# Zhang-Xiaoxue/Senquential-Convex-Programming-for-Trajectory-Planning

Measured on AMD Instinct MI355X. Metric: SCP-QP solves/sec/GPU (4 veh, Hp=20); traj ℓ∞ err vs CVXOPT, higher is better.
Workload: dtype f64; 1 GPU; c2: 4-vehicle circle/crossing, Hp=20, batch=1024 noise seeds per GPU, full SCP solve per problem; n_veh=4, hp=20, batch_per_gpu=1024, parallelism=1 independent shards (no collective)

## Files before the change

senquential-convex-programming-for-trajectory-planning_amd/csrc/scpqp_kernel.h:

```cpp

#pragma once

#include <hip/hip_runtime.h>

#include <math.h>
#include <stdint.h>
#include <stdio.h>
#include <stdlib.h>
#include <string.h>

#include <new>
#include <type_traits>
#include <utility>

#include "scpqp.h"

#define NT 256
#define TXD 16
#define TYD (NT / TXD)
#define NWAVE (NT / 64)
#define SCR_PER_WAVE 640

namespace {

// ... 1208 lines not shown
            if (u2 == 1 && tb == t) break;
            const int i0 = r1 + 2 * ia[u2], k0 = r1 + 2 * ka[u2];
            const int o0 = roff(i0), o1 = roff(i0 + 1);
            const double f = NEUTRAL ? 0.0 : 1.0;
            H[o0 + k0] -= f * sm[u2][0];
            H[o0 + k0 + 1] -= f * sm[u2][1];
            H[o1 + k0] -= f * sm[u2][2];
            H[o1 + k0 + 1] -= f * sm[u2][3];
        }
    }
}

typedef double double4v __attribute__((ext_vector_type(4)));

template <int U, int KS, class HP>
__device__ __forceinline__ void trailing_update_mfma(HP H, int n, int j0, int r1, const ldouble* dcur,
                                                     int wave, int nwave, int part = 0, int np = 1) {
    const int lane = threadIdx.x & 63, lr = lane & 15, lk = lane >> 4;
    double dk[KS];
#pragma unroll
    for (int kk = 0; kk < KS; ++kk) dk[kk] = dcur[4 * kk + lk];
    const int T = (n - r1 + 15) >> 4;
    const int ntile = T * (T + 1) / 2;
    int tb = 0, te = ntile;
    if (part != 0) {
        int js = 1, cum = T;
        for (int k = 1; k < np; ++k) {
            while (js < T && np * cum < k * ntile) {
                cum += T - js;
                ++js;
            }
            if (k == part - 1) tb = cum;
            if (k == part) te = cum;
        }
    }
    for (int t = tb + wave; t < te; t += U * nwave) {
        double a[U][KS], b[U][KS];
        double4v acc[U];
        int oc[U][4];
        bool ok[U][4];
#pragma unroll
        for (int u = 0; u < U; ++u) {
            const int tu = t + u * nwave;
            const bool live = tu < te;
            int I = 0, J = 0;
            tri_decode(ntile - 1 - (live ? tu : t), J, I);
            I = T - 1 - I;
            J = T - 1 - J;
            const int i0 = r1 + 16 * I, k0 = r1 + 16 * J;
            const int ia = min(i0 + lr, n - 1), kb = min(k0 + lr, n - 1);
            const int oa = roff(ia) + j0, ob = roff(kb) + j0;
#pragma unroll
            for (int kk = 0; kk < KS; ++kk) {
                a[u][kk] = -H[oa + 4 * kk + lk] * dk[kk];
                b[u][kk] = H[ob + 4 * kk + lk];
            }
            const int kc = k0 + lr;
#pragma unroll
            for (int r = 0; r < 4; ++r) {
                const int ci = i0 + lk + 4 * r;
                ok[u][r] = live && ci < n && kc <= ci;
                oc[u][r] = roff(ok[u][r] ? ci : 0) + (ok[u][r] ? kc : 0);
                acc[u][r] = ok[u][r] ? (double)H[oc[u][r]] : 0.0;
            }
        }
#pragma unroll
        for (int u = 0; u < U; ++u) {
#pragma unroll
            for (int kk = 0; kk < KS; ++kk)
                acc[u] = __builtin_amdgcn_mfma_f64_16x16x4f64(a[u][kk], b[u][kk], acc[u], 0, 0, 0);
        }
#pragma unroll
        for (int u = 0; u < U; ++u)
#pragma unroll
            for (int r = 0; r < 4; ++r)
                if (ok[u][r]) H[oc[u][r]] = acc[u][r];
    }
}

constexpr int kGroup = 4;
static_assert(kPivSlot + 2 * kGroup * CB == red_size(true) && kPivSlot + 2 * CB == red_size(false),
              "the pivot buffer of red_size");

template <class LT>
__device__ bool cholesky(const LT& L) {
    const int n = __builtin_amdgcn_readfirstlane(L.n);
    constexpr int RS = LT::RMAX;
    constexpr int G = LT::HGLOBAL ? kGroup : 1;
    lint* flag = (lint*)(L.red + kRedFlag);
    ldouble* ldbuf = L.red;
    ldouble* dbuf = L.red + kPivSlot;
    PROF_T0();
    for (int r0 = 0, s = 0; r0 < n; r0 += CB, ++s) {
        const int par = s & 1;
        const int jb = min(CB, n - r0), r1 = r0 + jb;
        const int sg = s % G;
        const int np = G == 1 ? 1 : (sg == 0 ? G : sg);
        const int jp = r0 - np * CB;
        const ldouble* dprev = dbuf + ((s - np) & (2 * G - 1)) * CB;
        if (is_lead(L.lead)) {
            ldouble* dn = dbuf + (s % (2 * G)) * CB;
            lead_prio_up();
            constexpr bool OPQ = RS > 2;
            if (RS == 1 || n - r0 <= 64) panel_factor<1, OPQ>(L.H, L.dinv, n, r0, jb, jp, dprev, dn, flag + par, np, ldbuf);
            else panel_factor<RS, OPQ>(L.H, L.dinv, n, r0, jb, jp, dprev, dn, flag + par, np, ldbuf);
            lead_prio_down();
        } else if (jp >= 0 || (G > 1 && s >= G)) {
            const int tw = (wave_id() - L.lead + NWAVE - 1) % NWAVE;
            if constexpr (LT::HGLOBAL) {
                constexpr int U = 2;
                const int s0 = s - sg;
                if (s0 >= G)
                    trailing_update_mfma<U, G * CB / 4>(L.H, n, (s0 - G) * CB, s0 * CB + CB,
                                                        dbuf + ((s0 - G) & (2 * G - 1)) * CB,
                                                        tw, NWAVE - 1, sg + 1, G);
            } else {
                trailing_update(L.H, n, jp, r1, dprev, tw * 64 + (int)(threadIdx.x & 63), NT - 64);
#ifdef SCPQP_DIAG_X2_TRAIL
                trailing_update<decltype(L.H), true>(L.H, n, jp, r1, dprev, tw * 64 + (int)(threadIdx.x & 63), NT - 64);
#endif
            }
        }
#if defined(SCPQP_PROF) && defined(SCPQP_PROF_FINE)
        unsigned long long _pb = __builtin_amdgcn_s_memtime();
#endif
        bar();
#if defined(SCPQP_PROF) && defined(SCPQP_PROF_FINE)
        if (threadIdx.x == 64 * L.lead) atomicAdd(&g_prof[22], __builtin_amdgcn_s_memtime() - _pb);
        if (threadIdx.x == 64 * ((L.lead + 1) & 3)) atomicAdd(&g_prof[23], __builtin_amdgcn_s_memtime() - _pb);
#endif
        if (flag[par]) return false;
    }
    PROF_ACC(13);
    return true;
}


constexpr int kSolveChunk = 4;
constexpr int kSolveChunkG = 8;
template <int LN, int LP>
__device__ __forceinline__ double bcast_capture_d(double v, double& dst, int& blo, int& bhi) {
    static_assert(LN >= 0 && LN < 64 && LP < 64, "lanes of the wave");
    const long long b = __double_as_longlong(v);
    const int vlo = static_cast<int>(b & 0xffffffffll), vhi = static_cast<int>(b >> 32);
    int lo, hi;
    if constexpr (LP >= 0) {
        const long long d = __double_as_longlong(dst);
        int dlo = static_cast<int>(d & 0xffffffffll), dhi = static_cast<int>(d >> 32);
        asm("s_nop 0\n\tv_readlane_b32 %0, %4, %8\n\tv_readlane_b32 %1, %5, %8\n\t"
            "v_writelane_b32 %2, %6, %9\n\tv_writelane_b32 %3, %7, %9"
            : "=&s"(lo), "=&s"(hi), "+v"(dlo), "+v"(dhi)
            : "v"(vlo), "v"(vhi), "s"(blo), "s"(bhi), "i"(LN), "i"(LP));
        dst = __longlong_as_double((static_cast<long long>(dhi) << 32) | static_cast<unsigned int>(dlo));
    } else {
        asm("s_nop 0\n\tv_readlane_b32 %0, %2, %4\n\tv_readlane_b32 %1, %3, %4\n\ts_nop 1"
            : "=&s"(lo), "=&s"(hi)
            : "v"(vlo), "v"(vhi), "i"(LN));
    }
    blo = lo;
    bhi = hi;
    return __longlong_as_double((static_cast<long long>(hi) << 32) | static_cast<unsigned int>(lo));
}
template <int LP>
__device__ __forceinline__ void flush_lane_d(double& dst, int blo, int bhi) {
    static_assert(LP >= 0 && LP < 64, "a lane of the wave");
    const long long d = __double_as_longlong(dst);
    int dlo = static_cast<int>(d & 0xffffffffll), dhi = static_cast<int>(d >> 32);
    asm("v_writelane_b32 %0, %2, %4\n\tv_writelane_b32 %1, %3, %4"
        : "+v"(dlo), "+v"(dhi)
        : "s"(blo), "s"(bhi), "i"(LP));
    dst = __longlong_as_double((static_cast<long long>(dhi) << 32) | static_cast<unsigned int>(dlo));
}
template <int R, class HP, int SCH, int NC = 0>
struct Solver {
    static constexpr bool RTN = NC == 0;
    static_assert(SCH % 2 == 0 && 64 % SCH == 0, "chunks tile the 64-row slots");
    static_assert(NC <= 64 * R, "every row has a slot");
    HP H;
    const ldouble* dinv;
    int lane, n, ld;
    double r[R], xf[R];
    int ii[R], ro[R], ic[R];
    double cur[R][SCH], nxt[R][SCH];

    __device__ __forceinline__ Solver(HP H_, const ldouble* dinv_, int n_, int ld_,
                                      const ldouble* bvec)
        : H(H_), dinv(dinv_), n(n_), ld(ld_) {
        lane = threadIdx.x & 63;
#pragma unroll
        for (int t = 0; t < R; ++t) {
            ii[t] = lane + 64 * t;
            ic[t] = ii[t] < n ? ii[t] : n - 1;
            ro[t] = roff(ic[t]);
            r[t] = ii[t] < n ? bvec[ii[t]] : 0.0;
            xf[t] = 0.0;
        }
    }
    __device__ __forceinline__ void load_cols(double (&dst)[R][SCH], int jc) {
#pragma unroll
        for (int t = 0; t < R; ++t)
#pragma unroll
            for (int q = 0; q < SCH; q += 2) {
                const double2v v = ld2(H + ro[t] + jc + q);
                dst[t][q] = v.x;
                dst[t][q + 1] = v.y;
            }
    }
    __device__ __forceinline__ void load_rows(double (&dst)[R][SCH], int jc) {
#pragma unroll
        for (int q = 0; q < SCH; ++q) {
            const int row = jc + q < n ? jc + q : n - 1;
#pragma unroll
            for (int t = 0; t < R; ++t) dst[t][q] = H[roff(row) + ic[t]];
        }
    }
// ... 25 lines not shown
    template <int T, int... C>
    __device__ __forceinline__ void fwd_chunks(std::integer_sequence<int, C...>) {
        (fwd_chunk<T, 64 * T + SCH * C>(std::make_integer_sequence<int, SCH>{}), ...);
    }
    template <int T, int J, int Q>
    __device__ __forceinline__ void bwd_step() {
        if constexpr (J < NC) {
            constexpr int jfirst = NC - 1 < 64 * T + 63 ? NC - 1 : 64 * T + 63;
            const double xj = bcast_capture_d<(J & 63), (J == jfirst ? -1 : ((J + 1) & 63))>(r[T], xf[T], blo, bhi);
            r[T] -= cur[T][Q] * xj;
#pragma unroll
            for (int t = 0; t < T; ++t) r[t] -= cur[t][Q] * xj;
        }
    }
    template <int T, int JC, int... Q>
    __device__ __forceinline__ void bwd_chunk(std::integer_sequence<int, Q...>) {
        if constexpr (JC > 0) load_rows(nxt, JC - SCH);
        (bwd_step<T, JC + SCH - 1 - Q, SCH - 1 - Q>(), ...);
        shift();
    }
    template <int T, int JSTART, int... C>
    __device__ __forceinline__ void bwd_chunks(std::integer_sequence<int, C...>) {
        (bwd_chunk<T, JSTART - SCH * C>(std::make_integer_sequence<int, SCH>{}), ...);
    }
    template <int T>
    __device__ __forceinline__ void fwd() {
        if constexpr (T < R && !RTN) {
            constexpr int jend = NC < 64 * (T + 1) ? NC : 64 * (T + 1);
            constexpr int nch = jend > 64 * T ? (jend - 64 * T + SCH - 1) / SCH : 0;
            fwd_chunks<T>(std::make_integer_sequence<int, nch>{});
            if constexpr (nch > 0) flush_lane_d<((jend - 1) & 63)>(xf[T], blo, bhi);
        } else if constexpr (T < R) {
            const int jend = min(n, 64 * (T + 1));
#pragma unroll 1
            for (int jc = 64 * T; jc < jend; jc += SCH) {
                if (jc + SCH < n) load_cols(nxt, jc + SCH);
#pragma unroll
                for (int q = 0; q < SCH; ++q) {
                    const int j = jc + q;
                    if (j < jend) {
                        const double xj = readlane_d(r[T], j & 63);
                        r[T] -= cur[T][q] * xj;
                        xf[T] = capture(xj, j, xf[T]);
#pragma unroll
                        for (int t = T + 1; t < R; ++t) r[t] -= cur[t][q] * xj;
                    }
                }
                shift();
            }
        }
    }
    template <int T>
    __device__ __forceinline__ void bwd(int jlast) {
        if constexpr (T < R && !RTN) {
            constexpr int jstart = (T == R - 1) ? ((NC - 1) / SCH) * SCH : 64 * T + 64 - SCH;
            constexpr int nch = jstart >= 64 * T ? (jstart - 64 * T) / SCH + 1 : 0;
            bwd_chunks<T, jstart>(std::make_integer_sequence<int, nch>{});
            if constexpr (nch > 0) flush_lane_d<0>(xf[T], blo, bhi);
        } else if constexpr (T < R) {
            const int jstart = (T == R - 1) ? jlast : 64 * T + 64 - SCH;
#pragma unroll 1
            for (int jc = jstart; jc >= 64 * T; jc -= SCH) {
                if (jc > 0) load_rows(nxt, jc - SCH);
#pragma unroll
                for (int q = SCH - 1; q >= 0; --q) {
                    const int j = jc + q;
                    if (j < n) {
                        const double xj = readlane_d(r[T], j & 63);
                        r[T] -= cur[T][q] * xj;
                        xf[T] = capture(xj, j, xf[T]);
#pragma unroll
                        for (int t = 0; t < T; ++t) r[t] -= cur[t][q] * xj;
                    }
                }
                shift();
            }
        }
    }
    __device__ __forceinline__ void run(ldouble* x) {
        PROF_T0();
        load_cols(cur, 0);
        fwd<0>(); fwd<1>(); fwd<2>(); fwd<3>();
        PROF_ACC(14);
#pragma unroll
        for (int t = 0; t < R; ++t) {
            r[t] = xf[t] * dinv[ic[t]];
            xf[t] = 0.0;
        }
        const int jlast = ((n - 1) / SCH) * SCH;
        load_rows(cur, jlast);
        bwd<3>(jlast); bwd<2>(jlast); bwd<1>(jlast); bwd<0>(jlast);
#pragma unroll
        for (int t = 0; t < R; ++t)
            if (ii[t] < n) x[ii[t]] = xf[t];
        PROF_ACC(15);
    }
};

template <int R, int NC, class LT>
__device__ __forceinline__ void chol_solve_r(const LT& L, const ldouble* bvec, ldouble* x) {
    Solver<R, decltype(L.H), (LT::HGLOBAL ? kSolveChunkG : kSolveChunk), NC> S(L.H, L.dinv, L.n, L.ld, bvec);
    S.run(x);
}

template <int SH, class LT>
__device__ void chol_solve(const LT& L, const ldouble* bvec, ldouble* x) {
    constexpr int NC = shape_c(SH).H == 0 ? 0 : shape_c(SH).V * shape_c(SH).H + 1;
#ifdef SCPQP_DIAG_X2_SOLVE
    for (int rep = 0; rep < 2; ++rep)
#endif
    if (is_lead(L.lead)) {
        constexpr int RM = LT::RMAX;
        lead_prio_up();
        if constexpr (NC != 0) {
            static_assert(NC <= 64 * RM, "the layout's row slots hold the shape");
            chol_solve_r<(NC + 63) / 64, NC>(L, bvec, x);
        } else {
            const int n = L.n;
            if (RM == 1 || n <= 64) chol_solve_r<1, 0>(L, bvec, x);
            else if (RM == 2 || n <= 128) chol_solve_r<(RM >= 2 ? 2 : 1), 0>(L, bvec, x);
            else if (RM == 3 || n <= 192) chol_solve_r<(RM >= 3 ? 3 : 1), 0>(L, bvec, x);
            else chol_solve_r<RM, 0>(L, bvec, x);
        }
        lead_prio_down();
    }
    bar();
}

struct EvalRes {
    double obj, maxv, sumv;
    int feasible;
};

__device__ __forceinline__ double d2_with_margin(double D, double margin) {
    const double Dm = D + margin;
    return __dmul_rn(Dm, Dm);
}

template <class LT>
__device__ EvalRes evaluate_u(const cParams& P, const LT& L, const ldouble* u, double* cveh,
                              double* cobs, const double* mg) {
    const int tid = threadIdx.x, V = L.V, Hb = L.Hb, O = L.O;
    toeplitz_apply(L, u, L.pb);
    bar();
    for (int e = tid; e < V * Hb; e += NT) {
        L.pb[2 * e] += L.p0[2 * e];
        L.pb[2 * e + 1] += L.p0[2 * e + 1];
    }
    bar();
    double obj = 0.0, mx = 0.0, sm = 0.0, nviol = 0.0;
    for (int e = tid; e < V * Hb; e += NT) {
        const int v = e / Hb, k = e % Hb;
        const double qk = (k == Hb - 1) ? P.Qf[v] : P.Q[v];
        const double ex = L.pb[2 * e] - L.ref[2 * e], ey = L.pb[2 * e + 1] - L.ref[2 * e + 1];
        obj += qk * (ex * ex + ey * ey) + P.R[v] * u[e] * u[e];
    }
    const bool quirk = (P.flags & SCPQP_FLAG_OBST_QUIRK) != 0;
    for (int r = tid; r < L.m; r += NT) {
        int i, j, o, k;
        row_decode(L.rinfo[r], i, j, o, k);
        const ldouble* pi = L.pb + (i * Hb + k) * 2;
        double dx, dy, D2;
        if (j >= 0) {
            dx = pi[0] - L.pb[(j * Hb + k) * 2];
            dy = pi[1] - L.pb[(j * Hb + k) * 2 + 1];
            D2 = P.D2veh[i * SCPQP_MAX_VEH + j];
        } else {
            dx = pi[0] - L.ob[(o * Hb + k) * 2];
            dy = pi[1] - L.ob[(o * Hb + k) * 2 + 1];
            D2 = P.D2obs[i * SCPQP_MAX_OBST + o];
            if (mg) D2 = d2_with_margin(P.Dobs[i * SCPQP_MAX_OBST + o], mg[o * Hb + k]);
        }
        const double c = D2 - (dx * dx + dy * dy);
        int reps = 1;
        if (j < 0 && quirk) reps = V - 1 - i;
        if (cveh && j >= 0) {
            cveh[(i * V + j) * Hb + k] = c;
            cveh[(j * V + i) * Hb + k] = c;
        }
        if (cobs && j < 0 && reps > 0) cobs[(i * O + o) * Hb + k] = c;
        if (c > P.ctol && reps > 0) {
            mx = fmax(mx, c);
            sm += c * reps;
            nviol += 1.0;
        }
    }
    double red[4] = {obj, sm, nviol, mx};
    block_reduce4<4>(red, 8, L.red);
    EvalRes res;
    res.obj = red[0];
    res.sumv = red[1];
    res.feasible = red[2] == 0.0;
    res.maxv = red[3];
    return res;
}

template <class LT>
__device__ void linearise_rows(const cParams& P, const LT& L, const double* mg) {
    const int tid = threadIdx.x, Hb = L.Hb;
    toeplitz_apply(L, L.ub, L.ya);
    bar();
    for (int e = tid; e < L.V * Hb; e += NT) {
        L.pb[2 * e] = L.p0[2 * e] + L.ya[2 * e];
        L.pb[2 * e + 1] = L.p0[2 * e + 1] + L.ya[2 * e + 1];
    }
    bar();
    for (int r = tid; r < L.m; r += NT) {
        int i, j, o, k;
        row_decode(L.rinfo[r], i, j, o, k);
// ... 186 lines not shown
    if (tid == 0) L.rd[N] = rdw;
    double red2[4] = {mrd, quad2, lin, 0.0};
    block_reduce4<3, 1>(red2, 1, L.red);
    out[0] = red[0];
    out[1] = fmax(red2[0], fabs(rdw));
    out[2] = red[1];
    out[3] = 0.5 * (red[3] + red2[1]) + red2[2] + P.slackW * zw;
}

struct Ctx {
    const cParams* P;
    gdouble* ws;
    int Hb, lead;
};
struct D4 {
    double a, b, c, d;
};

constexpr double kPolishTol = 1e-9;
__device__ __forceinline__ int polish_stop(const D4& d, int ref, double early) {
    if (ref < 1) return 0;
    if (d.a <= kPolishTol * fmax(1.0, d.b)) return 1;
    if (d.c > early || d.d > early) return 2;
    return 0;
}

__device__ __forceinline__ Ctx uniform_ctx(const Ctx& c) {
    Ctx u;
    u.P = (const cParams*)readfirstlane_u64((unsigned long long)c.P);
    u.ws = (gdouble*)readfirstlane_u64((unsigned long long)c.ws);
    u.Hb = __builtin_amdgcn_readfirstlane(c.Hb);
    u.lead = __builtin_amdgcn_readfirstlane(c.lead);
    return u;
}

template <bool HG, bool VG, int RM, int OCC, int SH>
__device__ __forceinline__ Lay<HG, VG, RM, OCC> lay_of(const Ctx& c) {
    const Off f = plan_offsets(shapeV<SH>(c.P->nV), shapeO<SH>(c.P->nO), shapeHM<SH>(c.P->hpMax), HG, VG, lean_plan(HG, VG, OCC));
    Lay<HG, VG, RM, OCC> L = make_lay<HG, VG, RM, OCC, SH>(lds_base(), c.ws, f, c.P->nV, c.P->nO, c.Hb);
    L.lead = c.lead;
    return L;
}
#define PHASE template <bool HG, bool VG, int RM, int OCC, int SH> __device__ __noinline__
#define LAYDEF                  \
    const Ctx cu_ = uniform_ctx(c); \
    const cParams& P = *cu_.P;  \
    const Lay<HG, VG, RM, OCC> L = lay_of<HG, VG, RM, OCC, SH>(cu_); \
    (void)P
#define PH(f) f<HG, VG, RM, OCC, SH>
#define ROWSDEF RowsOf<SH, Lay<HG, VG, RM, OCC>> A{L}

PHASE void ph_solve(Ctx c, int dst) {
    LAYDEF;
    chol_solve<SH>(L, L.rhs, dst ? L.dz : L.z);
}
template <int SH>
__device__ __forceinline__ const double* uniform_margin(const double* mg) {
    if constexpr (shape_c(SH).V != 0) return nullptr;
    else return (const double*)readfirstlane_u64((unsigned long long)mg);
}
PHASE int ph_margin_bad(Ctx c, const double* mg_) {
    LAYDEF;
    const double* mg = uniform_margin<SH>(mg_);
    lint* orslot = (lint*)(L.red + kOrSlot);
    if (threadIdx.x == 0) *orslot = 0;
    bar();
    bool bad = false;
    if (mg)
        for (int i = threadIdx.x; i < L.O * L.Hb; i += NT) bad |= !(mg[i] >= 0.0) || mg[i] == INFINITY;
    if (bad) *orslot = 1;
    bar();
    const int any = __builtin_amdgcn_readfirstlane(*orslot);
    bar();
    return any;
}
PHASE void ph_linearise(Ctx c, const double* mg) {
    LAYDEF;
    linearise_rows(P, L, uniform_margin<SH>(mg));
}
PHASE EvalRes ph_evaluate(Ctx c, double* cveh, double* cobs, const double* mg) {
    LAYDEF;
    return evaluate_u(P, L, L.ub, cveh, cobs, uniform_margin<SH>(mg));
}
PHASE D4 ph_residuals(Ctx c) {
    LAYDEF;
    ROWSDEF;
    A.template load<RV_S | RV_LAM>();
    double r[4];
    residuals(P, L, A, r);
    return D4{r[0], r[1], r[2], r[3]};
}
template <class LT>
__device__ __forceinline__ void rhs_from_tv_body(const cParams& P, const LT& L, double rho) {
    const double ow = gt_apply_fin<1>(L, L.tv, [&](int e, double g) { L.rhs[e] = g - L.qs[e] + rho * L.dz[e]; });
    if (threadIdx.x == 0) L.rhs[L.N] = ow - P.slackW + rho * L.dz[L.N];
    bar();
}
PHASE void ph_rhs_from_tv(Ctx c, double rho) {
    LAYDEF;
    rhs_from_tv_body(P, L, rho);
}
PHASE void ph_init_a(Ctx c) {
    LAYDEF;
    const int tid = threadIdx.x;
    for (int r = tid; r < L.mc; r += NT) {
        L.dd[r] = 1.0;
        L.tv[r] = hval(L, r);
    }
    for (int e = tid; e < L.n; e += NT) L.dz[e] = 0.0;
    bar();
}
PHASE void ph_init_b(Ctx c) {
    LAYDEF;
    const int tid = threadIdx.x, N = L.N, mc = L.mc;
    toeplitz_apply(L, L.z, L.ya);
    bar();
    double vmax = 0.0;
    for (int r = tid; r < L.m; r += NT) {
        const double gu = gx_row(L, L.z, 0.0, r);
        L.s[r] = gu;
        vmax = fmax(vmax, (gu - L.rowH[r]) / -L.rowW[r]);
    }
    double red[4] = {vmax, 0.0, 0.0, 0.0};
    block_reduce4<1>(red, 1, L.red);
    const double om = red[0] + 1.0;
    double smin = 1e300, smax = -1e300;
    for (int r = tid; r < mc; r += NT) {
        const double gx = r < L.m ? L.s[r] + L.rowW[r] * om : gx_row(L, L.z, om, r);
        const double sv = hval(L, r) - gx;
        L.s[r] = sv;
        smin = fmin(smin, sv);
        smax = fmax(smax, sv);
    }
    double red2[4] = {-smin, smax, 0.0, 0.0};
    block_reduce4<2, 1>(red2, 3, L.red);
    const double ts = fmax(1.5 * red2[0], 0.0);
    const double fl = 0.1 * fmax(1.0, red2[1] + ts);
    const double lam0 = 0.3 * P.slackW / mc;
    for (int r = tid; r < mc; r += NT) {
        L.s[r] = fmax(L.s[r] + ts, fl);
        L.lam[r] = r == mc - 1 ? P.slackW : lam0;
    }
    if (tid == 0) L.z[N] = om;
    bar();
}
template <bool TV = true, class LT, class RW>
__device__ __forceinline__ void newton_rhs_body(const LT& L, RW& A, int corr, double smu) {
    if constexpr (TV) {
        each_row(A, L.mc, [&](int k, int r) {
            const double rc = A.s(k, r) * A.lam(k, r) + (corr ? A.sa(k, r) * A.la(k, r) - smu : 0.0);
            L.tv[r] = A.dd(k, r) * A.rp(k, r) - rc * recip(A.s(k, r));
        });
        bar();
    }
    const double ow = gt_apply_fin<0>(L, L.tv, [&](int e, double g) { L.rhs[e] = -L.rd[e] - g; });
    if (threadIdx.x == 0) L.rhs[L.N] = -L.rd[L.N] - ow;
    bar();
}
template <class LT, class RW>
__device__ __forceinline__ double2v newton_back_body(const LT& L, RW& A, int corr, double smu) {
    toeplitz_apply(L, L.dz, L.ya);
    bar();
    const double xw = L.dz[L.N];
    double ap = 1.0, ad = 1.0;
    each_row(A, L.mc, [&](int k, int r) {
        const double rc = A.s(k, r) * A.lam(k, r) + (corr ? A.sa(k, r) * A.la(k, r) - smu : 0.0);
        const double dsr = -A.rp(k, r) - gx_row(L, L.dz, xw, r);
        const double dlr = -(rc + A.lam(k, r) * dsr) * recip(A.s(k, r));
        A.ds(k, r) = dsr;
        A.dl(k, r) = dlr;
        if (dsr < 0.0) ap = fmin(ap, -A.s(k, r) * recip(dsr));
        if (dlr < 0.0) ad = fmin(ad, -A.lam(k, r) * recip(dlr));
    });
    return double2v{ap, ad};
}
template <class LT, class RW>
__device__ __forceinline__ double affine_body(const LT& L, RW& A, double mu, double2v part) {
    double redm[4] = {-fmin(part.x, part.y), 0.0, 0.0, 0.0};
    block_reduce4<1>(redm, 1, L.red);
    const double aaff = -redm[0];
    double mua = 0.0;
    each_row(A, L.mc, [&](int k, int r) {
        mua += (A.s(k, r) + aaff * A.ds(k, r)) * (A.lam(k, r) + aaff * A.dl(k, r));
    });
    double red[4] = {mua, 0.0, 0.0, 0.0};
    block_reduce4<1, 1>(red, 0, L.red);
    const double sr = red[0] / L.mc / mu;
    return sr * sr * sr * mu;
}
template <class LT, class RW>
__device__ __forceinline__ void update_body(const LT& L, RW& A, double eta, double2v part) {
    double ap = part.x, ad = part.y;
    double red[4] = {-ap, -ad, 0.0, 0.0};
    block_reduce4<2>(red, 3, L.red);
    ap = fmin(1.0, eta * -red[0]);
    ad = fmin(1.0, eta * -red[1]);
    for (int e = threadIdx.x; e < L.n; e += NT) L.z[e] += ap * L.dz[e];
    each_row(A, L.mc, [&](int k, int r) {
        A.s(k, r) += ap * A.ds(k, r);
        A.lam(k, r) += ad * A.dl(k, r);
    });
    A.template store<RV_S | RV_LAM>();
    bar();
}
__device__ __forceinline__ double step_factor(double mu) { return fmax(0.99, 1.0 - mu); }
PHASE int ph_scale_assemble_rhs_factor(Ctx c) {
    LAYDEF;
    PROF_T0_FINE();
    assemble(P, L, L.dd, 0.0);
    PROF_ACC_FINE0(29);
    RowsMem<Lay<HG, VG, RM, OCC>> A{L};
    newton_rhs_body<false>(L, A, 0, 0.0);
    PROF_ACC_FINE0(28);
    return cholesky(L) ? 1 : 0;
}
PHASE int ph_assemble_factor(Ctx c, double rho) {
    LAYDEF;
    assemble(P, L, L.dd, rho);
    return cholesky(L) ? 1 : 0;
}
PHASE void ph_init_assemble_factor(Ctx c) {
    LAYDEF;
    assemble(P, L, L.dd, 0.0);
    const int N = L.N, o = roff(N);
    for (int e = threadIdx.x; e <= N; e += NT) L.H[o + e] = e == N ? 1.0 : 0.0;
    bar();
    cholesky(L);
}
PHASE double ph_back_affine_rhs(Ctx c, double mu) {
    LAYDEF;
    ROWSDEF;
    A.template load<RV_S | RV_LAM | RV_RP | RV_DD>();
    const double2v part = newton_back_body(L, A, 0, 0.0);
    const double smu = affine_body(L, A, mu, part);
    A.template store<RV_SA | RV_LA>();
    newton_rhs_body(L, A, 1, smu);
    return smu;
}
PHASE D4 ph_back_update_residuals(Ctx c, double smu, double eta) {
    LAYDEF;
    ROWSDEF;
    A.template load<RV_S | RV_LAM | RV_RP | RV_SA | RV_LA>();
    const double2v part = newton_back_body(L, A, 1, smu);
    update_body(L, A, eta, part);
    double r[4];
    residuals(P, L, A, r);
    return D4{r[0], r[1], r[2], r[3]};
}
PHASE void ph_polish_prep(Ctx c) {
    LAYDEF;
    const double idl = 1.0 / P.polDelta;
    if (threadIdx.x == 0) L.red[kIdlSlot] = idl;
    for (int r = threadIdx.x; r < L.mc; r += NT) {
        const bool act = L.lam[r] > L.s[r];
        L.dd[r] = act ? idl : 0.0;
        L.la[r] = act ? L.lam[r] : 0.0;
        L.sa[r] = act ? 1.0 : 0.0;
    }
    for (int e = threadIdx.x; e < L.n; e += NT) L.dz[e] = L.rd[e] = L.z[e];
    bar();
}
PHASE void ph_polish_warm(Ctx c) {
    LAYDEF;
    const double idl = 1.0 / P.polDelta;
    if (threadIdx.x == 0) L.red[kIdlSlot] = idl;
    for (int r = threadIdx.x; r < L.mc; r += NT) L.dd[r] = L.sa[r] != 0.0 ? idl : 0.0;
    for (int e = threadIdx.x; e < L.n; e += NT) L.dz[e] = L.rd[e] = L.z[e];
    bar();
}
PHASE D4 ph_scales(Ctx c) {
    LAYDEF;
    const int tid = threadIdx.x;
    double hmax = 1.0;
    for (int r = tid; r < L.m; r += NT) hmax = fmax(hmax, fabs(L.rowH[r]));
    double qmax = fmax(1.0, P.slackW);
    for (int e = tid; e < L.N; e += NT) qmax = fmax(qmax, fabs(L.qs[e]));
    double red[4] = {hmax, qmax, 0.0, 0.0};
    block_reduce4<2>(red, 3, L.red);
    return D4{red[0], red[1], 0.0, 0.0};
}
template <class LT, class RW>
__device__ __forceinline__ void polish_rhs_body(const cParams& P, const LT& L, RW& A) {
    const double idl = L.red[kIdlSlot];
    each_row(A, L.mc, [&](int k, int r) { L.tv[r] = A.sa(k, r) * (hval(L, r) * idl - A.la(k, r)); });
    bar();
    rhs_from_tv_body(P, L, P.polRho);
}
PHASE void ph_polish_rhs(Ctx c) {
    LAYDEF;
    ROWSDEF;
    A.template load<RV_SA | RV_LA>();
    polish_rhs_body(P, L, A);
}
template <class LT, class RW>
__device__ __forceinline__ D4 polish_dual_body(const cParams& P, const LT& L, RW& A) {
    const double idl = L.red[kIdlSlot];
    toeplitz_apply(L, L.dz, L.ya);
    bar();
    const double xw = L.dz[L.N];
    double viol = -1e300, yneg = -1e300;
    each_row(A, L.mc, [&](int k, int r) {
        const double hr = hval(L, r);
        const double rpr = gx_row(L, L.dz, xw, r) - hr;
        A.rp(k, r) = rpr;
        const double sar = A.sa(k, r);
        double y = A.la(k, r);
        if (sar != 0.0) {
            y = y + rpr * idl;
            A.la(k, r) = y;
            yneg = fmax(yneg, -y);
// ... 35 lines not shown
    }
    for (int e = tid; e < L.n; e += NT)
        if (!isfinite(L.dz[e])) nonfin = 1.0;
    double red[4] = {viol, -ymin, ymax, nonfin};
    block_reduce4<4, 1>(red, 15, L.red);
    const double vtol = 1e-9 * hmax, ytol = -1e-9 * fmax(1.0, red[2]);
    const bool ok = converged && red[0] <= vtol && -red[1] >= ytol && red[3] == 0.0;
    if (ok) {
        for (int e = tid; e < L.n; e += NT) L.z[e] = L.dz[e];
        bar();
        return 1;
    }
    if (red[3] != 0.0) return 0;
    const double idl = L.red[kIdlSlot];
    double changed = 0.0;
    for (int r = tid; r < L.mc; r += NT) {
        const bool act = L.sa[r] != 0.0;
        const bool add = !act && L.rp[r] > vtol;
        const bool drop = act && L.la[r] < ytol;
        if (add || drop) {
            changed += 1.0;
            L.sa[r] = add ? 1.0 : 0.0;
            L.la[r] = 0.0;
            L.dd[r] = add ? idl : 0.0;
        }
    }
    double red2[4] = {changed, 0.0, 0.0, 0.0};
    block_reduce4<1>(red2, 0, L.red);
    return red2[0] != 0.0 ? 1 + (int)red2[0] : 0;
}
PHASE void ph_take_u(Ctx c) {
    LAYDEF;
    for (int i = threadIdx.x; i < L.N; i += NT) L.ub[i] = P.uLim * L.z[i];
    bar();
}

PHASE void ph_trace_rows(Ctx c, double* dst) {
    LAYDEF;
    for (int i = threadIdx.x; i < L.N; i += NT) dst[kTraceHdr + i] = L.ub[i];
    const int N2 = kTraceHdr + 2 * P.nV * P.hpMax;
    for (int r = threadIdx.x; r < L.m; r += NT) {
        dst[N2 + 4 * r] = L.rowE[2 * r];
        dst[N2 + 4 * r + 1] = L.rowE[2 * r + 1];
        dst[N2 + 4 * r + 2] = L.rowW[r];
        dst[N2 + 4 * r + 3] = L.rowH[r];
    }
}
PHASE void ph_trace_sol(Ctx c, double* dst, D4 ev, double delta, int ipm, int qfl, double merit0,
                        int rounds, int refines) {
    LAYDEF;
    for (int i = threadIdx.x; i < L.N; i += NT) dst[kTraceHdr + P.nV * P.hpMax + i] = L.ub[i];
    if (threadIdx.x == 0) {
        dst[8] = merit0;
        dst[9] = rounds + 4096.0 * refines;
        dst[0] = delta;
        dst[1] = ev.a;
        dst[2] = ev.b;
        dst[3] = ev.c;
        dst[4] = L.z[L.N];
        dst[5] = ipm;
        dst[6] = qfl;
        dst[7] = ev.d;
    }
}

constexpr int kPolishRounds = 6;
constexpr int kWarmRounds = 8;
constexpr int kWarmRefine = 12;
constexpr double kWarmEarly = 1e-6;
constexpr bool kWarmStall = true;

struct QpStats {
    int ipm, rounds, refine, warm_ok;
};

template <bool HG, bool VG, int RM, int OCC, int SH>
__device__ __forceinline__ bool polish_rounds(Ctx c, double hmax, double rho, int max_rounds,
                                              int cap, double early, QpStats& st, bool stall = false) {
    bool ok = false, refactor = true, extended = false;
    int prev_chg = 1 << 30;
    PROF_T0();
    for (int round = 0; round < max_rounds && !ok; ++round) {
        ++st.rounds;
        if (refactor) {
            const bool fact = PH(ph_assemble_factor)(c, rho) != 0;
            PROF_ACC(7);
            if (!fact) break;
        }
        int conv = 0;
        PH(ph_polish_rhs)(c);
        for (int ref = 0; ref < cap; ++ref) {
            PH(ph_solve)(c, 1);
            const D4 d = PH(ph_polish_dual_next)(c, ref, cap, early);
            ++st.refine;
            const int stop = polish_stop(d, ref, early);
            conv = stop == 1;
            if (stop) break;
        }
        const int acc = PH(ph_polish_accept)(c, hmax, conv);
        PROF_ACC(8);
        ok = acc == 1;
        if (acc == 0 && (conv || extended)) break;
        if (acc >= 2) {
            if (stall && round >= 1 && acc - 1 >= prev_chg) break;
            prev_chg = acc - 1;
        }
        extended |= acc == 0;
        refactor = acc >= 2;
    }
    return ok;
}

struct QpKnobs {
    int maxIpm, nRefine, mc;
    double ipmTol, polRho;
};
template <bool HG, bool VG, int RM, int OCC, int SH>
__device__ __forceinline__ bool qp_solve_body(Ctx c, const QpKnobs& K, int& qflags, bool warm,
                                              QpStats& st) {
    const int mc = K.mc;
    const D4 sc = PH(ph_scales)(c);
    const double hmax = sc.a, qmax = sc.b;
    if (warm) {
        PH(ph_polish_warm)(c);
        if (polish_rounds<HG, VG, RM, OCC, SH>(c, hmax, K.polRho, kWarmRounds, kWarmRefine, kWarmEarly,
                                               st, kWarmStall)) {
            ++st.warm_ok;
            return true;
        }
    }
    PROF_T0();
    PH(ph_init_a)(c);
    PH(ph_init_assemble_factor)(c);
    PH(ph_rhs_from_tv)(c, 0.0);
    PH(ph_solve)(c, 0);
    PH(ph_init_b)(c);
    PROF_ACC(16);
    int it = 0;
    bool conv = false, ok = false, maxit = false;
    double tol = K.ipmTol;
    D4 res = PH(ph_residuals)(c);
    PROF_ACC(1);
    for (int pass = 0;; ++pass) {
        for (; it < K.maxIpm; ++it) {
            PROF_ACC(0);
            if (res.a <= tol * hmax && res.b <= tol * qmax && res.c <= tol * fmax(1.0, fabs(res.d))) {
                conv = true;
                break;
            }
            const double mu = res.c / mc;
            if (!PH(ph_scale_assemble_rhs_factor)(c)) break;
            PROF_ACC(3);
            PH(ph_solve)(c, 1);
            PROF_ACC(9);
            const double smu = PH(ph_back_affine_rhs)(c, mu);
            PROF_ACC(5);
            PH(ph_solve)(c, 1);
            PROF_ACC(9);
            res = PH(ph_back_update_residuals)(c, smu, step_factor(mu));
            PROF_ACC(6);
        }
        if (pass == 0 && !conv && it >= K.maxIpm) maxit = true;
        PH(ph_polish_prep)(c);
        ok = polish_rounds<HG, VG, RM, OCC, SH>(c, hmax, K.polRho, kPolishRounds, K.nRefine, INFINITY, st);
        if (ok || !conv || pass == 1) break;
        tol *= 0.01;
        conv = false;
        res = PH(ph_residuals)(c);
    }
    st.ipm += it;
    if (maxit) qflags |= SCPQP_FL_IPM_MAXIT;
    if (!ok) qflags |= SCPQP_FL_POLISH_REJECTED;
    return ok;
}
template <bool HG, bool VG, int RM, int OCC, int SH>
__device__ __noinline__ bool qp_solve(Ctx c0, int* qflags, bool warm, QpStats& st) {
    const Ctx c = uniform_ctx(c0);
    const cParams& P = *c.P;
    QpKnobs K;
    K.maxIpm = __builtin_amdgcn_readfirstlane(P.maxIpm);
    K.nRefine = __builtin_amdgcn_readfirstlane(P.nRefine);
    K.mc = __builtin_amdgcn_readfirstlane(
        (P.nV * (P.nV - 1) / 2 + P.nV * P.nO) * c.Hb + 2 * P.nV * c.Hb + 1);
    K.ipmTol = P.ipmTol;
    K.polRho = P.polRho;
    QpStats ls{0, 0, 0, 0};
    int lf = 0;
    const bool ok = qp_solve_body<HG, VG, RM, OCC, SH>(c, K, lf, warm, ls);
    st.ipm += ls.ipm;
    st.rounds += ls.rounds;
    st.refine += ls.refine;
    st.warm_ok += ls.warm_ok;
    *qflags |= lf;
    return ok;
}

__device__ unsigned g_cu_ctr[4096];
__device__ __forceinline__ int lead_wave_elect(lint* sh) {
    const unsigned hw = __builtin_amdgcn_s_getreg((31 << 11) | 4);
    const unsigned xcc = __builtin_amdgcn_s_getreg((3 << 11) | 20);
    const int simd = (hw >> 4) & 3;
    if (threadIdx.x == 0) {
        const unsigned key = ((xcc & 15) << 8) | (((hw >> 13) & 7) << 5) | (((hw >> 12) & 1) << 4) |
                             ((hw >> 8) & 15);
        sh[0] = atomicAdd(&g_cu_ctr[key], 1u) & 3;
        sh[1] = 0;
    }
    bar();
    if ((threadIdx.x & 63) == 0 && simd == sh[0]) sh[1] = threadIdx.x >> 6;
    bar();
    const int lead = __builtin_amdgcn_readfirstlane(sh[1]);
    bar();
    return lead;
}

template <bool HG, bool VG, int RM, int OCC, int SH>
__global__ __launch_bounds__(NT, OCC) void scp_kernel(KArgs a) {
    ldouble* smem = (ldouble*)smem_;
    const cParams& P0 = *(const cParams*)a.P;
    const int tid = threadIdx.x;
    gdouble* ws = a.ws ? (gdouble*)a.ws + (size_t)blockIdx.x * a.wsStride : nullptr;
    const Off f = plan_offsets(shapeV<SH>(P0.nV), shapeO<SH>(P0.nO), shapeHM<SH>(P0.hpMax), HG, VG, lean_plan(HG, VG, OCC));
    lint* slot = (lint*)(smem + f.red + kWorkSlot);
    lint* orslot = (lint*)(smem + f.red + kOrSlot);
    ldouble* lub = smem + f.ub;
    ldouble* lpb = smem + f.pb;
    ldouble* lref = smem + f.ref;
    ldouble* lg = smem + f.g;
    ldouble* lp0 = smem + f.p0;
    ldouble* lqs = smem + f.qs;
    const int lead = lead_wave_elect((lint*)(smem + f.red + kLeadSlot));
    for (;;) {
        if (tid == 0) {
            const int w = atomicAdd(a.counter, 1);
            slot[0] = (a.perm && w < a.B) ? a.perm[w] : w;
        }
// ... 229 lines not shown
```

senquential-convex-programming-for-trajectory-planning_amd/scpqp/build.py:

```python
from __future__ import annotations

import os
import shutil
import subprocess
import sys
import tempfile
from concurrent.futures import ThreadPoolExecutor

_PKG = os.path.dirname(os.path.abspath(__file__))
_ROOT = os.path.dirname(_PKG)
_REPO = os.path.dirname(_ROOT)
CSRC = os.path.join(_ROOT, "csrc")
SRC = os.path.join(CSRC, "scpqp.hip")
KERNEL_SRC = os.path.join(CSRC, "kernels.hip")
HEADER = os.path.join(CSRC, "scpqp_kernel.h")
SRCS = [SRC, os.path.join(CSRC, "plant.hip"), os.path.join(CSRC, "metrics.hip"),
        os.path.join(CSRC, "obstacles.hip"), os.path.join(CSRC, "sensing.hip"),
        os.path.join(CSRC, "estimator.hip"), os.path.join(CSRC, "tracker.hip"),
        os.path.join(CSRC, "manoeuvres.hip"), os.path.join(CSRC, "tracker_accel.hip"),
        os.path.join(CSRC, "imm.hip"), os.path.join(CSRC, "margin.hip")]
KERNEL_GROUPS = 10
INCLUDE = os.path.join(_REPO, "include")
LIB_PATH = os.path.join(_PKG, "libscpqp.so")
ARCH = os.environ.get("SCPQP_ARCH", "gfx950")


def _jobs():
    try:
        n = len(os.sched_getaffinity(0))
    except AttributeError:
        n = os.cpu_count() or 1
    return max(1, min(16, int(os.environ.get("MAX_JOBS", n)), n))


def build_library(force=False, verbose=False, defines=(), out=None, csrc=None):
    out = out or LIB_PATH
    src_dir = csrc or CSRC
    srcs = [os.path.join(src_dir, os.path.basename(x)) for x in SRCS]
    ksrc = os.path.join(src_dir, os.path.basename(KERNEL_SRC))
    hdr = os.path.join(src_dir, os.path.basename(HEADER))
    deps = srcs + [ksrc, hdr, os.path.join(src_dir, "scpqp_philox.h"),
                   os.path.join(src_dir, "scpqp_obstacle_pose.h"),
                   os.path.join(src_dir, "scpqp_manoeuvre_pose.h"),
                   os.path.join(src_dir, "scpqp_bicycle.h"),
                   os.path.join(INCLUDE, "scpqp_manoeuvres.h"),
                   os.path.join(INCLUDE, "scpqp_obstacles.h"),
                   os.path.join(INCLUDE, "scpqp_sensing.h"),
                   os.path.join(INCLUDE, "scpqp_estimator.h"),
                   os.path.join(INCLUDE, "scpqp_tracker.h"),
                   os.path.join(INCLUDE, "scpqp_tracker_accel.h"),
                   os.path.join(INCLUDE, "scpqp_imm.h"),
                   os.path.join(INCLUDE, "scpqp_margin.h"),
                   os.path.join(INCLUDE, "scpqp.h"), os.path.join(INCLUDE, "scpqp_noise.h"),
                   os.path.join(INCLUDE, "scpqp_metrics.h"),
                   os.path.join(INCLUDE, "scpqp_variants.h"),
                   os.path.join(INCLUDE, "scpqp_truth.h"), __file__]
    if not force and os.path.exists(out):
        t = os.path.getmtime(out)
        if all(os.path.getmtime(d) <= t for d in deps):
            return out
    flags = ["--offload-arch=" + ARCH, "-O3", "-std=c++17", "-fPIC", "-Wno-unused-result",
             f"-I{INCLUDE}"] + [f"-D{d}" for d in defines]
    tmp = tempfile.mkdtemp(prefix="scpqp_build_")
    try:
        units = [(s, os.path.join(tmp, os.path.basename(s) + ".o"), []) for s in srcs]
        units += [(ksrc, os.path.join(tmp, f"kernels_{g}.o"), [f"-DSCPQP_KGROUP={g}"])
                  for g in range(1, KERNEL_GROUPS + 1)]

        def compile_unit(u):
            src, obj, extra = u
            cmd = ["hipcc", "-c"] + flags + extra + [src, "-o", obj]
            if verbose:
                print(" ".join(cmd), file=sys.stderr)
            subprocess.run(cmd, check=True)
            return obj

        order = sorted(units, key=lambda u: 0 if u[2] and u[2][0].endswith(("=3", "=2", "=4")) else 1)
        with ThreadPoolExecutor(_jobs()) as ex:
            objs = list(ex.map(compile_unit, order))
        cmd = ["hipcc", "-shared", "-fPIC", "--offload-arch=" + ARCH] + objs + ["-o", out + ".tmp"]
        if verbose:
            print(" ".join(cmd), file=sys.stderr)
        subprocess.run(cmd, check=True)
        os.replace(out + ".tmp", out)
    finally:
        shutil.rmtree(tmp, ignore_errors=True)
    return out


if __name__ == "__main__":
    if "--prof" in sys.argv:
        defs = ("SCPQP_PROF", "SCPQP_PROF_FINE") if "--fine" in sys.argv else ("SCPQP_PROF",)
        print(build_library(force="--force" in sys.argv, verbose=True, defines=defs,
                            out=os.path.join(_PKG, "libscpqp_prof.so")))
    elif "--check" in sys.argv:
        print(build_library(force="--force" in sys.argv, verbose=True,
                            defines=("SCPQP_DIAG_REDUCE_CHECK",),
                            out=os.path.join(_PKG, "libscpqp_check.so")))
        print(build_library(force="--force" in sys.argv, verbose=True,
                            defines=("SCPQP_DIAG_REDUCE2",),
                            out=os.path.join(_PKG, "libscpqp_reduce2.so")))
    else:
        print(build_library(force="--force" in sys.argv, verbose=True))
```

Measured before the change: 143,600 SCP solves/s.

## Overlap forward triangular solve with Cholesky factorization on a helper wave

For the LDS-resident factor path, a helper wave now runs the forward substitution column block by column block during the Cholesky trailing-update steps, as soon as each panel is finished. The later solve only does the back substitution from the stored intermediate. Phases are merged so assembly, RHS construction, factorization and the forward solve happen in one call, which removes separate solve launches and barriers in the interior-point and polish loops. The cost is extra register pressure and work on one trailing-update wave, plus more complex control flow with edge cases when n mod CB equals 1.

```diff
diff --git a/senquential-convex-programming-for-trajectory-planning_amd/csrc/scpqp_kernel.h b/senquential-convex-programming-for-trajectory-planning_amd/csrc/scpqp_kernel.h
--- a/senquential-convex-programming-for-trajectory-planning_amd/csrc/scpqp_kernel.h
+++ b/senquential-convex-programming-for-trajectory-planning_amd/csrc/scpqp_kernel.h
@@ -1314,15 +1314,86 @@
 static_assert(kPivSlot + 2 * kGroup * CB == red_size(true) && kPivSlot + 2 * CB == red_size(false),
               "the pivot buffer of red_size");
 
-template <class LT>
-__device__ bool cholesky(const LT& L) {
+template <int RS, class HP>
+struct FwdPipe {
+    HP H;
+    int lane, n;
+    double r[RS], xf[RS];
+    int ro[RS];
+    __device__ __forceinline__ FwdPipe(HP H_, int n_) : H(H_), n(n_) {
+        lane = threadIdx.x & 63;
+#pragma unroll
+        for (int t = 0; t < RS; ++t) {
+            const int i = lane + 64 * t;
+            ro[t] = roff(i < n ? i : n - 1);
+            r[t] = xf[t] = 0.0;
+        }
+    }
+    __device__ __forceinline__ void load(const ldouble* b) {
+#pragma unroll
+        for (int t = 0; t < RS; ++t)
+            if (lane + 64 * t < n) r[t] = b[lane + 64 * t];
+    }
+    template <int T>
+    __device__ __forceinline__ void cols_t(int j0, int nc) {
+        if constexpr (T < RS) {
+            double cur[RS][CB];
+#pragma unroll
+            for (int t = T; t < RS; ++t)
+#pragma unroll
+                for (int q = 0; q < CB; q += 2) {
+                    const double2v v = ld2(H + ro[t] + j0 + q);
+                    cur[t][q] = v.x;
+                    cur[t][q + 1] = v.y;
+                }
+#pragma unroll
+            for (int q = 0; q < CB; ++q) {
+                const int j = j0 + q;
+                if (q < nc) {
+                    const double xj = readlane_d(r[T], j & 63);
+                    r[T] -= cur[T][q] * xj;
+                    xf[T] = (lane == (j & 63)) ? xj : xf[T];
+#pragma unroll
+                    for (int t = T + 1; t < RS; ++t) r[t] -= cur[t][q] * xj;
+                }
+            }
+        }
+    }
+    __device__ __forceinline__ void cols(int j0, int nc) {
+        const int T = j0 >> 6;
+        if (T == 0) cols_t<0>(j0, nc);
+        else if (T == 1) cols_t<1>(j0, nc);
+        else if (T == 2) cols_t<2>(j0, nc);
+        else cols_t<3>(j0, nc);
+    }
+    __device__ __forceinline__ void last_row(int j) {
+#pragma unroll
+        for (int t = 0; t < RS; ++t) xf[t] = (lane + 64 * t == j) ? r[t] : xf[t];
+    }
+    __device__ __forceinline__ void store(ldouble* y) const {
+#pragma unroll
+        for (int t = 0; t < RS; ++t)
+            if (lane + 64 * t < n) y[lane + 64 * t] = xf[t];
+    }
+};
+
+template <int ROLE, class LT>
+__device__ __forceinline__ bool cholesky_steps(const LT& L, const ldouble* b, ldouble* y) {
     const int n = __builtin_amdgcn_readfirstlane(L.n);
     constexpr int RS = LT::RMAX;
+    static_assert(RS <= 4, "FwdPipe::cols dispatches four row slots");
     constexpr int G = LT::HGLOBAL ? kGroup : 1;
+    constexpr bool PIPE = !LT::HGLOBAL;
+    static_assert(PIPE == (ROLE != 2), "split step loops with an LDS factor only");
+    const bool helper = ROLE == 1 && b != nullptr && wave_id() == (L.lead + 1) % NWAVE;
+    FwdPipe<ROLE == 1 ? RS : 1, decltype(L.H)> fp(L.H, n);
+    if constexpr (ROLE == 1) {
+        if (helper) fp.load(b);
+    }
     lint* flag = (lint*)(L.red + kRedFlag);
     ldouble* ldbuf = L.red;
     ldouble* dbuf = L.red + kPivSlot;
-    PROF_T0();
+#pragma unroll 1
     for (int r0 = 0, s = 0; r0 < n; r0 += CB, ++s) {
         const int par = s & 1;
         const int jb = min(CB, n - r0), r1 = r0 + jb;
@@ -1330,7 +1401,7 @@
         const int np = G == 1 ? 1 : (sg == 0 ? G : sg);
         const int jp = r0 - np * CB;
         const ldouble* dprev = dbuf + ((s - np) & (2 * G - 1)) * CB;
-        if (is_lead(L.lead)) {
+        if (ROLE == 0 || (ROLE == 2 && is_lead(L.lead))) {
             ldouble* dn = dbuf + (s % (2 * G)) * CB;
             lead_prio_up();
             constexpr bool OPQ = RS > 2;
@@ -1351,6 +1422,13 @@
 #ifdef SCPQP_DIAG_X2_TRAIL
                 trailing_update<decltype(L.H), true>(L.H, n, jp, r1, dprev, tw * 64 + (int)(threadIdx.x & 63), NT - 64);
 #endif
+                if (helper) {
+                    fp.cols(jp, CB);
+                    if (jb == 1) {
+                        fp.last_row(r0);
+                        fp.store(y);
+                    }
+                }
             }
         }
 #if defined(SCPQP_PROF) && defined(SCPQP_PROF_FINE)
@@ -1363,6 +1441,25 @@
 #endif
         if (flag[par]) return false;
     }
+    if constexpr (PIPE) {
+        if (b != nullptr && !(n % CB == 1 && n > CB)) {
+            if (helper) {
+                const int rl = ((n - 1) / CB) * CB;
+                fp.cols(rl, n - rl);
+                fp.store(y);
+            }
+            bar();
+        }
+    }
+    return true;
+}
+template <class LT>
+__device__ bool cholesky(const LT& L, const ldouble* b = nullptr, ldouble* y = nullptr) {
+    PROF_T0();
+    bool ok;
+    if constexpr (LT::HGLOBAL) ok = cholesky_steps<2>(L, b, y);
+    else ok = is_lead(L.lead) ? cholesky_steps<0>(L, b, y) : cholesky_steps<1>(L, b, y);
+    if (!ok) return false;
     PROF_ACC(13);
     return true;
 }
@@ -1554,9 +1651,15 @@
         load_cols(cur, 0);
         fwd<0>(); fwd<1>(); fwd<2>(); fwd<3>();
         PROF_ACC(14);
+        back<true>(x);
+    }
+    __device__ __forceinline__ void run_from_y(ldouble* x) { back<false>(x); }
+    template <bool YXF>
+    __device__ __forceinline__ void back(ldouble* x) {
+        PROF_T0();
 #pragma unroll
         for (int t = 0; t < R; ++t) {
-            r[t] = xf[t] * dinv[ic[t]];
+            r[t] = (YXF ? xf[t] : r[t]) * dinv[ic[t]];
             xf[t] = 0.0;
         }
         const int jlast = ((n - 1) / SCH) * SCH;
@@ -1569,34 +1672,46 @@
     }
 };
 
-template <int R, int NC, class LT>
+template <int R, int NC, bool FROMY, class LT>
 __device__ __forceinline__ void chol_solve_r(const LT& L, const ldouble* bvec, ldouble* x) {
     Solver<R, decltype(L.H), (LT::HGLOBAL ? kSolveChunkG : kSolveChunk), NC> S(L.H, L.dinv, L.n, L.ld, bvec);
-    S.run(x);
-}
-
-template <int SH, class LT>
+    if constexpr (FROMY) S.run_from_y(x);
+    else S.run(x);
+}
+
+template <int SH, bool FROMY = false, class LT>
 __device__ void chol_solve(const LT& L, const ldouble* bvec, ldouble* x) {
     constexpr int NC = shape_c(SH).H == 0 ? 0 : shape_c(SH).V * shape_c(SH).H + 1;
 #ifdef SCPQP_DIAG_X2_SOLVE
-    for (int rep = 0; rep < 2; ++rep)
+    for (int rep = 0; rep < (FROMY ? 1 : 2); ++rep)
 #endif
     if (is_lead(L.lead)) {
         constexpr int RM = LT::RMAX;
         lead_prio_up();
         if constexpr (NC != 0) {
             static_assert(NC <= 64 * RM, "the layout's row slots hold the shape");
-            chol_solve_r<(NC + 63) / 64, NC>(L, bvec, x);
+            chol_solve_r<(NC + 63) / 64, NC, FROMY>(L, bvec, x);
         } else {
             const int n = L.n;
-            if (RM == 1 || n <= 64) chol_solve_r<1, 0>(L, bvec, x);
-            else if (RM == 2 || n <= 128) chol_solve_r<(RM >= 2 ? 2 : 1), 0>(L, bvec, x);
-            else if (RM == 3 || n <= 192) chol_solve_r<(RM >= 3 ? 3 : 1), 0>(L, bvec, x);
-            else chol_solve_r<RM, 0>(L, bvec, x);
+            if (RM == 1 || n <= 64) chol_solve_r<1, 0, FROMY>(L, bvec, x);
+            else if (RM == 2 || n <= 128) chol_solve_r<(RM >= 2 ? 2 : 1), 0, FROMY>(L, bvec, x);
+            else if (RM == 3 || n <= 192) chol_solve_r<(RM >= 3 ? 3 : 1), 0, FROMY>(L, bvec, x);
+            else chol_solve_r<RM, 0, FROMY>(L, bvec, x);
         }
         lead_prio_down();
     }
     bar();
+}
+
+template <int SH, class LT>
+__device__ __forceinline__ bool factor_solve(const LT& L, ldouble* x) {
+    if constexpr (LT::HGLOBAL) {
+        return cholesky(L);
+    } else {
+        if (!cholesky(L, L.rhs, x)) return false;
+        chol_solve<SH, true>(L, x, x);
+        return true;
+    }
 }
 
 struct EvalRes {
@@ -1949,6 +2064,10 @@
     LAYDEF;
     return evaluate_u(P, L, L.ub, cveh, cobs, uniform_margin<SH>(mg));
 }
+PHASE void ph_rhs_from_tv(Ctx c, double rho) {
+    LAYDEF;
+    rhs_from_tv_body(P, L, rho);
+}
 PHASE D4 ph_residuals(Ctx c) {
     LAYDEF;
     ROWSDEF;
@@ -1962,10 +2081,6 @@
     const double ow = gt_apply_fin<1>(L, L.tv, [&](int e, double g) { L.rhs[e] = g - L.qs[e] + rho * L.dz[e]; });
     if (threadIdx.x == 0) L.rhs[L.N] = ow - P.slackW + rho * L.dz[L.N];
     bar();
-}
-PHASE void ph_rhs_from_tv(Ctx c, double rho) {
-    LAYDEF;
-    rhs_from_tv_body(P, L, rho);
 }
 PHASE void ph_init_a(Ctx c) {
     LAYDEF;
@@ -2079,20 +2194,26 @@
     RowsMem<Lay<HG, VG, RM, OCC>> A{L};
     newton_rhs_body<false>(L, A, 0, 0.0);
     PROF_ACC_FINE0(28);
-    return cholesky(L) ? 1 : 0;
-}
-PHASE int ph_assemble_factor(Ctx c, double rho) {
+    return factor_solve<SH>(L, L.dz) ? 1 : 0;
+}
+PHASE int ph_polish_rhs_assemble_factor(Ctx c, double rho) {
     LAYDEF;
     assemble(P, L, L.dd, rho);
-    return cholesky(L) ? 1 : 0;
-}
-PHASE void ph_init_assemble_factor(Ctx c) {
+    if constexpr (!HG) {
+        ROWSDEF;
+        A.template load<RV_SA | RV_LA>();
+        polish_rhs_body(P, L, A);
+    }
+    return factor_solve<SH>(L, L.dz) ? 1 : 0;
+}
+PHASE int ph_init_rhs_assemble_factor(Ctx c) {
     LAYDEF;
     assemble(P, L, L.dd, 0.0);
     const int N = L.N, o = roff(N);
     for (int e = threadIdx.x; e <= N; e += NT) L.H[o + e] = e == N ? 1.0 : 0.0;
-    bar();
-    cholesky(L);
+    if constexpr (HG) bar();
+    else rhs_from_tv_body(P, L, 0.0);
+    return factor_solve<SH>(L, L.z) ? 1 : 0;
 }
 PHASE double ph_back_affine_rhs(Ctx c, double mu) {
     LAYDEF;
@@ -2294,15 +2415,18 @@
     PROF_T0();
     for (int round = 0; round < max_rounds && !ok; ++round) {
         ++st.rounds;
+        bool solved = false;
         if (refactor) {
-            const bool fact = PH(ph_assemble_factor)(c, rho) != 0;
+            const bool fact = PH(ph_polish_rhs_assemble_factor)(c, rho) != 0;
             PROF_ACC(7);
             if (!fact) break;
-        }
+            solved = !HG;
+        }
+        if (HG || !refactor) PH(ph_polish_rhs)(c);
         int conv = 0;
-        PH(ph_polish_rhs)(c);
         for (int ref = 0; ref < cap; ++ref) {
-            PH(ph_solve)(c, 1);
+            if (!solved) PH(ph_solve)(c, 1);
+            solved = false;
             const D4 d = PH(ph_polish_dual_next)(c, ref, cap, early);
             ++st.refine;
             const int stop = polish_stop(d, ref, early);
@@ -2343,9 +2467,13 @@
     }
     PROF_T0();
     PH(ph_init_a)(c);
-    PH(ph_init_assemble_factor)(c);
-    PH(ph_rhs_from_tv)(c, 0.0);
-    PH(ph_solve)(c, 0);
+    const bool fact0 = PH(ph_init_rhs_assemble_factor)(c) != 0;
+    if constexpr (HG) {
+        PH(ph_rhs_from_tv)(c, 0.0);
+        PH(ph_solve)(c, 0);
+    } else if (!fact0) {
+        PH(ph_solve)(c, 0);
+    }
     PH(ph_init_b)(c);
     PROF_ACC(16);
     int it = 0;
@@ -2363,7 +2491,7 @@
             const double mu = res.c / mc;
             if (!PH(ph_scale_assemble_rhs_factor)(c)) break;
             PROF_ACC(3);
-            PH(ph_solve)(c, 1);
+            if constexpr (HG) PH(ph_solve)(c, 1);
             PROF_ACC(9);
             const double smu = PH(ph_back_affine_rhs)(c, mu);
             PROF_ACC(5);
diff --git a/senquential-convex-programming-for-trajectory-planning_amd/scpqp/build.py b/senquential-convex-programming-for-trajectory-planning_amd/scpqp/build.py
--- a/senquential-convex-programming-for-trajectory-planning_amd/scpqp/build.py
+++ b/senquential-convex-programming-for-trajectory-planning_amd/scpqp/build.py
@@ -33,7 +33,7 @@
     return max(1, min(16, int(os.environ.get("MAX_JOBS", n)), n))
 
 
-def build_library(force=False, verbose=False, defines=(), out=None, csrc=None):
+def build_library(force=False, verbose=False, defines=(), out=None, csrc=None, extra_flags=()):
     out = out or LIB_PATH
     src_dir = csrc or CSRC
     srcs = [os.path.join(src_dir, os.path.basename(x)) for x in SRCS]
@@ -60,7 +60,7 @@
         if all(os.path.getmtime(d) <= t for d in deps):
             return out
     flags = ["--offload-arch=" + ARCH, "-O3", "-std=c++17", "-fPIC", "-Wno-unused-result",
-             f"-I{INCLUDE}"] + [f"-D{d}" for d in defines]
+             f"-I{INCLUDE}"] + [f"-D{d}" for d in defines] + list(extra_flags)
     tmp = tempfile.mkdtemp(prefix="scpqp_build_")
     try:
         units = [(s, os.path.join(tmp, os.path.basename(s) + ".o"), []) for s in srcs]
```

Result: no change. 143,500 SCP solves/s (median of 5 runs) (-0.0%).
